# ZhangXinWhut/SimWhisper-Codec

Hardware: AMD Instinct MI355X
Metric: audio-sec/sec encode+decode (RTF^-1), 16kHz batch=32x10s (higher is better)
Workload: dtype split-f16 x3 encode (f32-class, f32 accumulate) / bf16 decode (f32 accumulate); 1 GPU; batch=32x10s @16kHz per GPU (32 utterances in all), encode()+decode(), 0.1*N(0,1) seed 1234, synthetic closed-form checkpoint (291M params); precision=mixed

## Files before the change

simwhisper_codec_amd/csrc/swc_gemm.hip:

```cpp
#include "swc_common.h"

static inline int tuning_env(const char* name, int dflt = 0) {
#ifdef SWC_TUNING
    const char* e = getenv(name);
    return e ? atoi(e) : dflt;
#else
    (void)name;
    return dflt;
#endif
}

namespace {


__device__ __attribute__((aligned(16))) unsigned int g_zero16[4] = {0u, 0u, 0u, 0u};
#ifdef SWC_GEMM_STAMP
__device__ unsigned long long g_stamps[512 * 8 * 8];
#endif

__device__ __forceinline__ void glds16(const void* gsrc, unsigned lds_addr) {
    unsigned keep;
    lds_addr = __builtin_amdgcn_readfirstlane(lds_addr);
    asm volatile(
        "s_mov_b32 %0, m0\n\ts_mov_b32 m0, %2\n\ts_nop 0\n\tglobal_load_lds_dwordx4 %1, off\n\ts_mov_b32 m0, %0"
        : "=&s"(keep)
        : "v"(gsrc), "s"(lds_addr)
        : "memory");
}
__device__ __forceinline__ void glds16_s(const char* base, unsigned off, unsigned lds_addr) {
    unsigned keep;
    lds_addr = __builtin_amdgcn_readfirstlane(lds_addr);
    asm volatile(
        "s_mov_b32 %0, m0\n\ts_mov_b32 m0, %3\n\ts_nop 0\n\tglobal_load_lds_dwordx4 %1, %2\n\ts_mov_b32 m0, %0"
        : "=&s"(keep)
        : "v"(off), "s"(base), "s"(lds_addr)
        : "memory");
}
__device__ __forceinline__ unsigned lds_addr_of(const void* p) {
    return (unsigned)(uintptr_t)(const __attribute__((address_space(3))) char*)p;
}

__device__ __forceinline__ int swz(int row) { return ((row >> 1) ^ ((row >> 4) << 1)) & 7; }
__device__ __forceinline__ int swz64(int row) { return ((-(row >> 2)) ^ (-(row >> 4))) & 3; }
template <int RB>
__device__ __forceinline__ int swz_rb(int row) { return RB == 128 ? swz(row) : swz64(row); }
template <int RB>
__device__ __forceinline__ int lds_off(int row, int chunk) { return row * RB + ((chunk ^ swz_rb<RB>(row)) << 4); }


struct GemmP {
    const char* A;
    const char* W;
    void* C;
    const float* bias;
    const float* gamma;
    const float* residual;
    long lda, ldw, ldc, ldr;
    int M, N, K;
    int taps, dil, stride, pad, t_in, t_out;
    int act;
    float alpha, out_scale;
    int band;
    unsigned* sat;
    int kc_per_tap;
    int n_tiles_n, n_tiles_m;
    int nt_mode;
    int stagger;
};

constexpr int EPI_TP = 68;
constexpr int EPI_WAVE_BYTES = 16 * EPI_TP * 4;


typedef unsigned u32x4_t __attribute__((ext_vector_type(4)));
typedef unsigned u32x2_t __attribute__((ext_vector_type(2)));
__device__ __forceinline__ void epi_st128(void* p, unsigned a, unsigned b, unsigned c, unsigned d, bool nt = false) {
#if defined(SWC_ABL_NOSTORE)
    asm volatile("" ::"v"(p), "v"(a), "v"(b), "v"(c), "v"(d));
#elif defined(SWC_EPI_PLAIN)
    (void)nt;
    *reinterpret_cast<uint4*>(p) = make_uint4(a, b, c, d);
#else
    if (nt) __builtin_nontemporal_store((u32x4_t){a, b, c, d}, reinterpret_cast<u32x4_t*>(p));
    else *reinterpret_cast<uint4*>(p) = make_uint4(a, b, c, d);
#endif
}
__device__ __forceinline__ void epi_st128f(void* p, float a, float b, float c, float d, bool nt = false) {
    epi_st128(p, __float_as_uint(a), __float_as_uint(b), __float_as_uint(c), __float_as_uint(d), nt);
}
__device__ __forceinline__ void epi_st64(void* p, unsigned a, unsigned b, bool nt = false) {
#if defined(SWC_ABL_NOSTORE)
    asm volatile("" ::"v"(p), "v"(a), "v"(b));
#elif defined(SWC_EPI_PLAIN)
    (void)nt;
    *reinterpret_cast<uint2*>(p) = make_uint2(a, b);
#else
    if (nt) __builtin_nontemporal_store((u32x2_t){a, b}, reinterpret_cast<u32x2_t*>(p));
    else *reinterpret_cast<uint2*>(p) = make_uint2(a, b);
#endif
}
__device__ __forceinline__ void epi_st32(void* p, unsigned a, bool nt = false) {
#if defined(SWC_ABL_NOSTORE)
    asm volatile("" ::"v"(p), "v"(a));
#elif defined(SWC_EPI_PLAIN)
    (void)nt;
    *reinterpret_cast<unsigned*>(p) = a;
#else
    if (nt) __builtin_nontemporal_store(a, reinterpret_cast<unsigned*>(p));
    else *reinterpret_cast<unsigned*>(p) = a;
#endif
}

template <typename OutT>
__device__ __forceinline__ float epi_act(float x) {
    return (__is_same(OutT, bf16_t) || __is_same(OutT, fp8_t)) ? gelu_fast(x) : (__is_same(OutT, f16s_t) ? gelu_as(x) : gelu_erf(x));
}

template <typename OutT, int MT, bool GELU>
__device__ __forceinline__ void gemm_epilogue_slab(const GemmP& p, f32x4 (&acc)[MT][4], int row0, int colw, int fr, int fh,
                                                   float* tbuf, float& amax, bool nt) {
    int lane = fr + 16 * fh;
    asm volatile("" : "+v"(lane));
    const int tr = lane >> 4, tc = (lane & 15) * 4;
    const int col = colw + tc;
    float4 b4 = make_float4(0.f, 0.f, 0.f, 0.f), g4 = make_float4(1.f, 1.f, 1.f, 1.f);
    if (p.bias) b4 = *reinterpret_cast<const float4*>(p.bias + col);
    if (p.gamma) g4 = *reinterpret_cast<const float4*>(p.gamma + col);
    float* wr_p = tbuf + (lane & 15) * EPI_TP + (lane >> 4) * 16;
    const float* rd_p = tbuf + tr * EPI_TP + tc;
#ifndef SWC_EPI_RD
#define SWC_EPI_RD 2
#endif
    constexpr int RD = SWC_EPI_RD < MT ? SWC_EPI_RD : MT - 1;
    float4 r4[MT][4];
    auto load_res = [&](int i) {
#pragma unroll
        for (int k = 0; k < 4; ++k) {
            const int row = row0 + 16 * i + tr + 4 * k;
            r4[i][k] = row < p.M ? *reinterpret_cast<const float4*>(p.residual + (long)row * p.ldr + col) : make_float4(0.f, 0.f, 0.f, 0.f);
        }
    };
    if (p.residual) {
#pragma unroll
        for (int i = 0; i < RD; ++i) load_res(i);
    }
#pragma unroll
    for (int i = 0; i < MT; ++i) {
        const int rbase = row0 + 16 * i + tr;
        if (p.residual && i + RD < MT) load_res(i + RD);
#pragma unroll
        for (int j = 0; j < 4; ++j) *reinterpret_cast<f32x4*>(wr_p + 4 * j) = acc[i][j];
        f32x4 t[4];
#pragma unroll
        for (int k = 0; k < 4; ++k) t[k] = *reinterpret_cast<const f32x4*>(rd_p + 4 * k * EPI_TP);
#pragma unroll
        for (int k = 0; k < 4; ++k) {
            const int row = rbase + 4 * k;
            float v0 = t[k][0] * p.alpha + b4.x, v1 = t[k][1] * p.alpha + b4.y, v2 = t[k][2] * p.alpha + b4.z, v3 = t[k][3] * p.alpha + b4.w;
            if constexpr (GELU) { v0 = epi_act<OutT>(v0); v1 = epi_act<OutT>(v1); v2 = epi_act<OutT>(v2); v3 = epi_act<OutT>(v3); }
            v0 *= g4.x; v1 *= g4.y; v2 *= g4.z; v3 *= g4.w;
            if (p.residual) { v0 += r4[i][k].x; v1 += r4[i][k].y; v2 += r4[i][k].z; v3 += r4[i][k].w; }
            if (row >= p.M) continue;
            if constexpr (__is_same(OutT, f16s_t)) {
                const float os = p.out_scale;
                f16s_store4(reinterpret_cast<unsigned short*>(p.C) + (long)row * p.ldc * 2, col, v0 * os, v1 * os, v2 * os, v3 * os, amax);
            } else if constexpr (sizeof(OutT) == 4) {
                epi_st128f(reinterpret_cast<float*>(p.C) + (long)row * p.ldc + col, v0, v1, v2, v3, nt);
            } else if constexpr (sizeof(OutT) == 1) {
                const float os = p.out_scale;
                epi_st32(reinterpret_cast<unsigned char*>(p.C) + (long)row * p.ldc + col, fp8_pack4(v0 * os, v1 * os, v2 * os, v3 * os, amax), nt);
            } else {
                epi_st64(reinterpret_cast<bf16_t*>(p.C) + (long)row * p.ldc + col, bf16_pack2(v0, v1), bf16_pack2(v2, v3), nt);
            }
        }
    }
}

template <typename OutT, int MT, int GELU>
__device__ __forceinline__ void gemm_epilogue_direct(const GemmP& p, f32x4 (&acc)[MT][4], int bm, int bn, int wr, int wc, int fr,
                                                     int fh, bool nt) {
    OutT* C = reinterpret_cast<OutT*>(p.C);
    const int col0 = bn + wc * 64 + 16 * fh;
    const bool vec_ok = (col0 + 16 <= p.N) && ((p.ldc & (sizeof(OutT) == 1 ? 15 : 3)) == 0) &&
                        (!p.residual || (p.ldr & 3) == 0) &&
                        ((reinterpret_cast<uintptr_t>(p.C) & 15) == 0) &&
                        ((reinterpret_cast<uintptr_t>(p.residual) & 15) == 0);
#ifdef SWC_KEEP_GAMMA16
    constexpr bool HAS_GAMMA = true;
#else
    constexpr bool HAS_GAMMA = sizeof(OutT) == 4;
#endif
    float bv[16], gv[HAS_GAMMA ? 16 : 1];
    float amax = 0.f;
    (void)amax; (void)gv;
    if (col0 + 16 <= p.N && ((reinterpret_cast<uintptr_t>(p.bias) | reinterpret_cast<uintptr_t>(p.gamma)) & 15) == 0) {
#pragma unroll
        for (int q = 0; q < 4; ++q) {
            const float4 b4 = p.bias ? *reinterpret_cast<const float4*>(p.bias + col0 + 4 * q) : make_float4(0.f, 0.f, 0.f, 0.f);
            bv[4 * q] = b4.x; bv[4 * q + 1] = b4.y; bv[4 * q + 2] = b4.z; bv[4 * q + 3] = b4.w;
            if constexpr (HAS_GAMMA) {
                const float4 g4 = p.gamma ? *reinterpret_cast<const float4*>(p.gamma + col0 + 4 * q) : make_float4(1.f, 1.f, 1.f, 1.f);
                gv[4 * q] = g4.x; gv[4 * q + 1] = g4.y; gv[4 * q + 2] = g4.z; gv[4 * q + 3] = g4.w;
            }
        }
    } else {
#pragma unroll
        for (int c = 0; c < 16; ++c) {
            const int col = col0 + c;
            bv[c] = (p.bias && col < p.N) ? p.bias[col] : 0.f;
            if constexpr (HAS_GAMMA) gv[c] = (p.gamma && col < p.N) ? p.gamma[col] : 1.f;
        }
    }
#pragma unroll
    for (int i = 0; i < MT; ++i) {
        const int row = bm + wr * (MT * 16) + i * 16 + fr;
        if (row >= p.M) continue;
        float v[16];
#pragma unroll
        for (int j = 0; j < 4; ++j)
#pragma unroll
            for (int e = 0; e < 4; ++e) v[4 * j + e] = acc[i][j][e] * p.alpha + bv[4 * j + e];
        if constexpr (GELU == 1) {
#pragma unroll
            for (int c = 0; c < 16; ++c) v[c] = epi_act<OutT>(v[c]);
        } else if constexpr (GELU == 2) {
#pragma unroll
            for (int c = 0; c < 16; ++c)
                if (p.act == SWC_ACT_GELU) v[c] = epi_act<OutT>(v[c]);
        }
        if constexpr (HAS_GAMMA) {
#pragma unroll
            for (int c = 0; c < 16; ++c) v[c] *= gv[c];
        }
        if constexpr (sizeof(OutT) == sizeof(f16s_t) && !__is_same(OutT, bf16_t)) {
            if (col0 + 16 <= p.N) {
                if (p.residual) {
                    const float4* rp = reinterpret_cast<const float4*>(p.residual + (long)row * p.ldr + col0);
#pragma unroll
                    for (int j = 0; j < 4; ++j) {
                        const float4 r4 = rp[j];
                        v[4 * j] += r4.x; v[4 * j + 1] += r4.y; v[4 * j + 2] += r4.z; v[4 * j + 3] += r4.w;
                    }
                }
                unsigned short* rowp = reinterpret_cast<unsigned short*>(p.C) + (long)row * p.ldc * 2;
                unsigned h2[8], l2[8];
#pragma unroll
                for (int c = 0; c < 8; ++c) f16s_split2(v[2 * c] * p.out_scale, v[2 * c + 1] * p.out_scale, h2[c], l2[c], amax);
                unsigned short* hp = rowp + f16s_col(col0);
#pragma unroll
                for (int q = 0; q < 2; ++q) {
                    epi_st128(reinterpret_cast<uint4*>(hp) + q, h2[4 * q], h2[4 * q + 1], h2[4 * q + 2], h2[4 * q + 3], nt);
                    epi_st128(reinterpret_cast<uint4*>(hp + 32) + q, l2[4 * q], l2[4 * q + 1], l2[4 * q + 2], l2[4 * q + 3], nt);
                }
            }
        } else if (vec_ok) {
            if (p.residual) {
                const float4* rp = reinterpret_cast<const float4*>(p.residual + (long)row * p.ldr + col0);
#pragma unroll
                for (int j = 0; j < 4; ++j) {
                    const float4 r4 = rp[j];
                    v[4 * j] += r4.x; v[4 * j + 1] += r4.y; v[4 * j + 2] += r4.z; v[4 * j + 3] += r4.w;
                }
            }
            OutT* cp = C + (long)row * p.ldc + col0;
            if constexpr (sizeof(OutT) == 4) {
#pragma unroll
                for (int j = 0; j < 4; ++j)
                    epi_st128f(reinterpret_cast<float4*>(cp) + j, v[4 * j], v[4 * j + 1], v[4 * j + 2], v[4 * j + 3], nt);
            } else if constexpr (sizeof(OutT) == 1) {
                const float os = p.out_scale;
                const unsigned u0 = fp8_pack4(v[0] * os, v[1] * os, v[2] * os, v[3] * os, amax);
                const unsigned u1 = fp8_pack4(v[4] * os, v[5] * os, v[6] * os, v[7] * os, amax);
                const unsigned u2 = fp8_pack4(v[8] * os, v[9] * os, v[10] * os, v[11] * os, amax);
                const unsigned u3 = fp8_pack4(v[12] * os, v[13] * os, v[14] * os, v[15] * os, amax);
                epi_st128(cp, u0, u1, u2, u3, nt);
            } else {
#pragma unroll
                for (int j = 0; j < 2; ++j)
                    epi_st128(reinterpret_cast<uint4*>(cp) + j, bf16_pack2(v[8 * j + 0], v[8 * j + 1]), bf16_pack2(v[8 * j + 2], v[8 * j + 3]),
                              bf16_pack2(v[8 * j + 4], v[8 * j + 5]), bf16_pack2(v[8 * j + 6], v[8 * j + 7]), nt);
            }
        } else {
#pragma unroll
            for (int c = 0; c < 16; ++c) {
                const int col = col0 + c;
                if (col >= p.N) continue;
                float x = v[c];
                if (p.residual) x += p.residual[(long)row * p.ldr + col];
                if constexpr (__is_same(OutT, fp8_t)) { x *= p.out_scale; amax = fmaxf(amax, fabsf(x)); }
                if constexpr (!__is_same(OutT, f16s_t)) store_out<OutT>(C + (long)row * p.ldc + col, x);
            }
        }
    }
    if constexpr (__is_same(OutT, f16s_t)) sat_commit(p.sat, 0, amax, SWC_F16S_LIMIT);
    if constexpr (__is_same(OutT, fp8_t)) sat_commit(p.sat, 1, amax, SWC_FP8_LIMIT);
}

template <typename OutT, int MT, bool SLAB, int ACT>
__device__ __forceinline__ void gemm_epilogue(const GemmP& p, f32x4 (&acc)[MT][4], int bm, int bn, int wr, int wc, int fr,
                                              int fh, float* tbuf, bool nt) {
    const bool gelu = ACT == 1 || (ACT == 2 && p.act == SWC_ACT_GELU);
    if constexpr (SLAB && sizeof(OutT) == 4 && !__is_same(OutT, f16s_t)) {
        const int colw = bn + wc * 64;
        const bool al16 = ((reinterpret_cast<uintptr_t>(p.C) | reinterpret_cast<uintptr_t>(p.residual) |
                            reinterpret_cast<uintptr_t>(p.bias) | reinterpret_cast<uintptr_t>(p.gamma)) & 15) == 0;
        const bool ok = tbuf && colw + 64 <= p.N && al16 && (p.ldc & (sizeof(OutT) == 1 ? 15 : 3)) == 0 &&
                        (!p.residual || (p.ldr & 3) == 0);
        if (__builtin_amdgcn_readfirstlane((int)ok)) {
            float amax = 0.f;
            if (gelu) gemm_epilogue_slab<OutT, MT, true>(p, acc, bm + wr * (MT * 16), colw, fr, fh, tbuf, amax, nt);
            else gemm_epilogue_slab<OutT, MT, false>(p, acc, bm + wr * (MT * 16), colw, fr, fh, tbuf, amax, nt);
            if constexpr (__is_same(OutT, fp8_t)) sat_commit(p.sat, 1, amax, SWC_FP8_LIMIT);
            return;
        }
    }
    if constexpr (ACT != 2) {
        gemm_epilogue_direct<OutT, MT, ACT>(p, acc, bm, bn, wr, wc, fr, fh, nt);
    } else if constexpr (__is_same(OutT, f16s_t) && MT == 8) {
        gemm_epilogue_direct<OutT, MT, 2>(p, acc, bm, bn, wr, wc, fr, fh, nt);
    } else {
        if (gelu) gemm_epilogue_direct<OutT, MT, 1>(p, acc, bm, bn, wr, wc, fr, fh, nt);
        else gemm_epilogue_direct<OutT, MT, 0>(p, acc, bm, bn, wr, wc, fr, fh, nt);
    }
}

template <int MODE, typename OutT, int MT, int WAVES_M, int WAVES_N, bool PLAIN, int RB = 128, int ACT = 2>
__global__ __launch_bounds__(WAVES_M* WAVES_N * 64, 2) void gemm_kernel(GemmP p) {
    constexpr int ROW_BYTES = RB;
    constexpr int CPR = RB / 16;
    constexpr int NG = RB / 64;
    static_assert(RB == 128 || (RB == 64 && MODE != SWC_F16S), "split-f16 needs hi|lo in one 128-byte row");
    static_assert(WAVES_M * WAVES_N * EPI_WAVE_BYTES <= (WAVES_M * MT * 16 + WAVES_N * 64) * RB, "epilogue scratch must fit one stage");
    constexpr bool BF16 = MODE == SWC_BF16;
    constexpr bool F16S = MODE == SWC_F16S;
    constexpr bool FP8 = MODE == SWC_FP8;
    constexpr int ES = BF16 ? 2 : (FP8 ? 1 : 4);
    constexpr int EPC = 16 / ES;
    constexpr int BK = ROW_BYTES / ES;
    constexpr int NT = WAVES_M * WAVES_N * 64;
    constexpr int BM = WAVES_M * MT * 16;
    constexpr int BN = WAVES_N * 64;
    constexpr int RPS = NT / CPR;
    constexpr int NA = BM / RPS;
    constexpr int NB = BN / RPS;
    constexpr int A_BYTES = BM * ROW_BYTES;
    constexpr int STAGE_BYTES = (BM + BN) * ROW_BYTES;

    extern __shared__ __attribute__((aligned(16))) char smem[];

    const int tid = threadIdx.x;
    const int lane = tid & 63;
    const int wave = tid >> 6;
    const int wr = wave / WAVES_N, wc = wave % WAVES_N;

    const int ntiles = p.n_tiles_m * p.n_tiles_n;
    const int xcd = blockIdx.x & 7;
    const int gw = ((int)gridDim.x - xcd + 7) >> 3;
    const int cq = ntiles >> 3, cr = ntiles & 7;
    const int chunk_start = xcd < cr ? xcd * (cq + 1) : cr * (cq + 1) + (xcd - cr) * cq;
    const int chunk_size = cq + (xcd < cr ? 1 : 0);
    int tl = blockIdx.x >> 3;
    if (tl >= chunk_size) return;
    int bm, bn;
    auto tile_origin = [&](int local) {
        const int bid = chunk_start + local;
        const int BAND = p.band;
        const int band = bid / (BAND * p.n_tiles_n);
        const int rem = bid - band * (BAND * p.n_tiles_n);
        const int rows_in_band = (p.n_tiles_m - band * BAND) < BAND ? (p.n_tiles_m - band * BAND) : BAND;
        const int tn = rem / rows_in_band;
        const int tm = band * BAND + (rem - tn * rows_in_band);
        bm = tm * BM;
        bn = tn * BN;
    };

    const int ld_pos = tid % CPR;
    const int ld_row = tid / CPR;
    int a_b[NA], a_t[NA], a_chunk[NA];
    bool a_rowok[NA];
    long w_rowoff[NB];
    int w_chunk[NB];
    bool w_rowok[NB];
    const int wave_u = __builtin_amdgcn_readfirstlane(wave);
    const unsigned smem_base = __builtin_amdgcn_readfirstlane(lds_addr_of(smem));
    constexpr int NV = RPS >= 64 ? 1 : 64 / RPS;
    unsigned chunkoff[NV];
#pragma unroll
    for (int v = 0; v < NV; ++v) chunkoff[v] = (unsigned)(ld_pos ^ swz_rb<RB>(ld_row + RPS * v)) << 4;
    const unsigned lda_bytes = (unsigned)(p.lda * ES), ldw_bytes = (unsigned)(p.ldw * ES);
    const char* a_base = p.A;
    const char* w_base = p.W;
    int a_left = 1, w_left = 1;
    auto setup_tile = [&](int local) {
        tile_origin(local);
        if constexpr (PLAIN) {
            a_base = p.A + (long)bm * lda_bytes;
            w_base = p.W + (long)bn * ldw_bytes;
            a_left = p.M - bm;
            w_left = p.N - bn;
            return;
        }
#pragma unroll
        for (int i = 0; i < NA; ++i) {
            const int row = ld_row + RPS * i;
            const int r = bm + row;
            const int chunk = ld_pos ^ swz_rb<RB>(row);
            if constexpr (!PLAIN) {
                a_rowok[i] = r < p.M;
                const int rr = a_rowok[i] ? r : 0;
                a_b[i] = rr / p.t_out;
                a_t[i] = rr - a_b[i] * p.t_out;
                a_chunk[i] = chunk;
            }
        }
#pragma unroll
        for (int i = 0; i < NB; ++i) {
            const int row = ld_row + RPS * i;
            const int n = bn + row;
            const int chunk = ld_pos ^ swz_rb<RB>(row);
            if constexpr (!PLAIN) {
                w_rowok[i] = n < p.N;
                w_rowoff[i] = (long)(w_rowok[i] ? n : 0) * p.ldw;
                w_chunk[i] = chunk;
            }
        }
    };
    setup_tile(tl);
    if (p.stagger > 0) {
        const int phase = (blockIdx.x >> 3) & 7;
        if (phase) {
            const unsigned long long t0 = __builtin_amdgcn_s_memtime();
            const unsigned long long wait = (unsigned long long)phase * (unsigned)p.stagger;
            while (__builtin_amdgcn_s_memtime() - t0 < wait) __builtin_amdgcn_s_sleep(32);
        }
    }
    auto stage_slice = [&](int kt, int stage) {
        const unsigned sa = smem_base + stage * STAGE_BYTES + wave_u * 1024;
        const unsigned sb = sa + A_BYTES;
        if constexpr (PLAIN) {
            const long koff = (long)kt * ROW_BYTES;
            const char* ab = a_base + koff;
            const char* wb = w_base + koff;
#pragma unroll
            for (int i = 0; i < NA; ++i) {
                const int r = min(ld_row + RPS * i, a_left - 1);
                glds16_s(ab, __umul24(r, lda_bytes) + chunkoff[i % NV], sa + RPS * i * ROW_BYTES);
            }
#pragma unroll
            for (int i = 0; i < NB; ++i) {
                const int r = min(ld_row + RPS * i, w_left - 1);
                glds16_s(wb, __umul24(r, ldw_bytes) + chunkoff[i % NV], sb + RPS * i * ROW_BYTES);
            }
            return;
        }
        const int tap = kt / p.kc_per_tap;
        const int kc = kt - tap * p.kc_per_tap;
        const int shift = tap * p.dil - p.pad;
        const char* zero = reinterpret_cast<const char*>(g_zero16);
#pragma unroll
        for (int i = 0; i < NA; ++i) {
            const int k0 = kc * BK + a_chunk[i] * EPC;
            const int ts = a_t[i] * p.stride + shift;
            const bool ok = a_rowok[i] && k0 < p.K && ts >= 0 && ts < p.t_in;
            const char* src = p.A + (((long)a_b[i] * p.t_in + (ok ? ts : 0)) * p.lda + (ok ? k0 : 0)) * ES;
            glds16(ok ? src : zero, sa + RPS * i * ROW_BYTES);
        }
#pragma unroll
        for (int i = 0; i < NB; ++i) {
            const int k0 = kc * BK + w_chunk[i] * EPC;
            const bool ok = w_rowok[i] && k0 < p.K;
            const char* src = p.W + (w_rowoff[i] + (long)tap * p.K + (ok ? k0 : 0)) * ES;
            glds16(ok ? src : zero, sb + RPS * i * ROW_BYTES);
        }
    };
#ifdef SWC_GEMM_STAMP
    unsigned long long st_last = 0, st_cmp = 0, st_vm = 0, st_bar = 0, st_n = 0;
    auto stamp = [&]() -> unsigned long long {
        unsigned long long t;
        asm volatile("s_memtime %0\n\ts_waitcnt lgkmcnt(0)" : "=s"(t)::"memory");
        return t;
    };
    auto dma_fence = [&]() {
        asm volatile("s_waitcnt lgkmcnt(0)" ::: "memory");
        const unsigned long long t1 = stamp();
        asm volatile("s_waitcnt vmcnt(0)" ::: "memory");
        const unsigned long long t2 = stamp();
        __syncthreads();
        const unsigned long long t3 = stamp();
        if (st_last) { st_cmp += t1 - st_last; st_vm += t2 - t1; st_bar += t3 - t2; st_n += 1; }
        st_last = t3;
    };
#else
    auto dma_fence = [&]() {
        asm volatile("s_waitcnt vmcnt(0)" ::: "memory");
        __syncthreads();
    };
#endif

    f32x4 acc[MT][4];
#pragma unroll
    for (int i = 0; i < MT; ++i)
#pragma unroll
        for (int j = 0; j < 4; ++j) acc[i][j] = (f32x4){0.f, 0.f, 0.f, 0.f};

    const int nkt = p.taps * p.kc_per_tap;
    const int fr = lane & 15, fh = lane >> 4;
    const int a_row0 = wr * (MT * 16) + fr;
    const int b_row0 = wc * 64 + 16 * (fr >> 2) + (fr & 3);
    stage_slice(0, 0);
    dma_fence();
#ifdef SWC_GEMM_PRIO47
    if (wave_u >= (WAVES_M * WAVES_N) / 2) __builtin_amdgcn_s_setprio(1);
#endif
    for (;;) {
    for (int kt = 0; kt < nkt; ++kt) {
        const int cur = kt & 1;
        if (kt + 1 < nkt) stage_slice(kt + 1, cur ^ 1);
#ifdef SWC_GEMM_IGLP
        __builtin_amdgcn_iglp_opt(SWC_GEMM_IGLP);
#endif
        const char* sa = smem + cur * STAGE_BYTES;
        const char* sb = sa + A_BYTES;
#ifdef SWC_GEMM_SPLIT
        constexpr bool EXPLICIT_SPLIT = (BF16 || F16S) && WAVES_M * WAVES_N == 8 && MT >= 4;
        constexpr int SPLIT = SWC_GEMM_SPLIT;
#else
        constexpr bool EXPLICIT_SPLIT = (F16S && WAVES_M * WAVES_N == 8 && MT >= 4) || ((BF16 || F16S) && WAVES_M * WAVES_N == 4);
        constexpr int SPLIT = WAVES_M * WAVES_N == 4 ? 0 : (MT == 8 ? 3 : 1);
#endif
        if constexpr (EXPLICIT_SPLIT) {
            uint4 f0a[MT], f0b[4], f1a[MT], f1b[4];
#pragma unroll
            for (int j = 0; j < 4; ++j) f0b[j] = *reinterpret_cast<const uint4*>(sb + lds_off<RB>(b_row0 + 4 * j, fh));
#pragma unroll
            for (int i = 0; i < MT; ++i) f0a[i] = *reinterpret_cast<const uint4*>(sa + lds_off<RB>(a_row0 + 16 * i, fh));
#pragma unroll
            for (int j = 0; j < 4; ++j) f1b[j] = *reinterpret_cast<const uint4*>(sb + lds_off<RB>(b_row0 + 4 * j, fh + 4));
#pragma unroll
            for (int i = 0; i < MT; ++i) f1a[i] = *reinterpret_cast<const uint4*>(sa + lds_off<RB>(a_row0 + 16 * i, fh + 4));
            auto mm = [&](int i) {
#pragma unroll
                for (int j = 0; j < 4; ++j) {
                    f32x4 c = acc[i][j];
                    if constexpr (F16S) {
                        c = __builtin_amdgcn_mfma_f32_16x16x32_f16(*reinterpret_cast<f16x8*>(&f1b[j]), *reinterpret_cast<f16x8*>(&f0a[i]), c, 0, 0, 0);
                        c = __builtin_amdgcn_mfma_f32_16x16x32_f16(*reinterpret_cast<f16x8*>(&f0b[j]), *reinterpret_cast<f16x8*>(&f1a[i]), c, 0, 0, 0);
                        c = __builtin_amdgcn_mfma_f32_16x16x32_f16(*reinterpret_cast<f16x8*>(&f0b[j]), *reinterpret_cast<f16x8*>(&f0a[i]), c, 0, 0, 0);
                    } else {
                        c = __builtin_amdgcn_mfma_f32_16x16x32_bf16(*reinterpret_cast<bf16x8*>(&f0b[j]), *reinterpret_cast<bf16x8*>(&f0a[i]), c, 0, 0, 0);
                        c = __builtin_amdgcn_mfma_f32_16x16x32_bf16(*reinterpret_cast<bf16x8*>(&f1b[j]), *reinterpret_cast<bf16x8*>(&f1a[i]), c, 0, 0, 0);
                    }
                    acc[i][j] = c;
                }
            };
#pragma unroll
            for (int i = 0; i < MT - SPLIT; ++i) mm(i);
            __builtin_amdgcn_sched_barrier(0);
            dma_fence();
            __builtin_amdgcn_sched_barrier(0);
#pragma unroll
            for (int i = MT - SPLIT; i < MT; ++i) mm(i);
            continue;
        }
        uint4 ha[(F16S || FP8) ? MT : 1], hb[(F16S || FP8) ? 4 : 1];
        (void)ha; (void)hb;
#pragma unroll
        for (int g = 0; g < NG; ++g) {
            uint4 fa[MT], fb[4];
#pragma unroll
            for (int j = 0; j < 4; ++j)
                fb[j] = *reinterpret_cast<const uint4*>(sb + lds_off<RB>(b_row0 + 4 * j, fh + 4 * g));
#pragma unroll
            for (int i = 0; i < MT; ++i)
                fa[i] = *reinterpret_cast<const uint4*>(sa + lds_off<RB>(a_row0 + 16 * i, fh + 4 * g));
            if constexpr (F16S) {
                if (g == 0) {
#pragma unroll
                    for (int i = 0; i < MT; ++i) ha[i] = fa[i];
#pragma unroll
                    for (int j = 0; j < 4; ++j) hb[j] = fb[j];
                } else {
#pragma unroll
                    for (int i = 0; i < MT; ++i)
#pragma unroll
                        for (int j = 0; j < 4; ++j) {
                            f32x4 c = acc[i][j];
                            c = __builtin_amdgcn_mfma_f32_16x16x32_f16(*reinterpret_cast<f16x8*>(&fb[j]),
                                                                       *reinterpret_cast<f16x8*>(&ha[i]), c, 0, 0, 0);
                            c = __builtin_amdgcn_mfma_f32_16x16x32_f16(*reinterpret_cast<f16x8*>(&hb[j]),
                                                                       *reinterpret_cast<f16x8*>(&fa[i]), c, 0, 0, 0);
                            c = __builtin_amdgcn_mfma_f32_16x16x32_f16(*reinterpret_cast<f16x8*>(&hb[j]),
                                                                       *reinterpret_cast<f16x8*>(&ha[i]), c, 0, 0, 0);
                            acc[i][j] = c;
                        }
                }
            } else if constexpr (BF16) {
#pragma unroll
                for (int i = 0; i < MT; ++i)
#pragma unroll
                    for (int j = 0; j < 4; ++j)
                        acc[i][j] = __builtin_amdgcn_mfma_f32_16x16x32_bf16(
                            *reinterpret_cast<bf16x8*>(&fb[j]), *reinterpret_cast<bf16x8*>(&fa[i]), acc[i][j], 0, 0, 0);
            } else if constexpr (FP8) {
                if (g == 0) {
#pragma unroll
                    for (int i = 0; i < MT; ++i) ha[i] = fa[i];
#pragma unroll
                    for (int j = 0; j < 4; ++j) hb[j] = fb[j];
                } else {
#pragma unroll
                    for (int i = 0; i < MT; ++i)
#pragma unroll
                        for (int j = 0; j < 4; ++j) {
                            i32x8 wa, xa;
                            wa[0] = hb[j].x; wa[1] = hb[j].y; wa[2] = hb[j].z; wa[3] = hb[j].w;
                            wa[4] = fb[j].x; wa[5] = fb[j].y; wa[6] = fb[j].z; wa[7] = fb[j].w;
                            xa[0] = ha[i].x; xa[1] = ha[i].y; xa[2] = ha[i].z; xa[3] = ha[i].w;
                            xa[4] = fa[i].x; xa[5] = fa[i].y; xa[6] = fa[i].z; xa[7] = fa[i].w;
                            acc[i][j] = __builtin_amdgcn_mfma_scale_f32_16x16x128_f8f6f4(wa, xa, acc[i][j], 0, 0, 0, 0x7f7f7f7f, 0,
                                                                                         0x7f7f7f7f);
                        }
                }
            } else {
#pragma unroll
                for (int e = 0; e < 4; ++e)
#pragma unroll
                    for (int i = 0; i < MT; ++i) {
                        const float av = __uint_as_float(reinterpret_cast<const unsigned*>(&fa[i])[e]);
#pragma unroll
                        for (int j = 0; j < 4; ++j) {
                            const float bv = __uint_as_float(reinterpret_cast<const unsigned*>(&fb[j])[e]);
                            acc[i][j] = __builtin_amdgcn_mfma_f32_16x16x4f32(bv, av, acc[i][j], 0, 0, 0);
                        }
                    }
            }
        }
        dma_fence();
    }
    const int bm_done = bm, bn_done = bn;
    tl += gw;
    const bool more = tl < chunk_size;
    if (more) {
        setup_tile(tl);
        stage_slice(0, 0);
    }
#ifdef SWC_GEMM_STAMP
    const unsigned long long st_e0 = stamp();
#endif
    gemm_epilogue<OutT, MT, MT < 8, ACT>(p, acc, bm_done, bn_done, wr, wc, fr, fh,
                            reinterpret_cast<float*>(smem + STAGE_BYTES + wave_u * EPI_WAVE_BYTES),
                            p.nt_mode == 2 || (p.nt_mode == 1 && !more));
#ifdef SWC_GEMM_STAMP
    asm volatile("s_waitcnt vmcnt(0)" ::: "memory");
    const unsigned long long st_e1 = stamp();
    if (lane == 0 && blockIdx.x < 512) {
        unsigned long long* o = g_stamps + ((long)blockIdx.x * 8 + wave) * 8;
        o[0] += st_cmp; o[1] += st_vm; o[2] += st_bar; o[3] += st_n; o[4] += st_e1 - st_e0; o[5] += 1; o[6] += st_e0 - st_last;
    }
    st_cmp = st_vm = st_bar = st_n = 0; st_last = 0;
#endif
    if (!more) break;
#pragma unroll
    for (int i = 0; i < MT; ++i)
#pragma unroll
        for (int j = 0; j < 4; ++j) acc[i][j] = (f32x4){0.f, 0.f, 0.f, 0.f};
    dma_fence();
    }
}

template <int MODE, typename OutT, int MT, int WM, int WN, bool PLAIN, int RB = 128, int ACT = 2>
int launch_k(GemmP p, hipStream_t s) {
    constexpr int BM = WM * MT * 16, BN = WN * 64;
    constexpr int LDS = 2 * (BM + BN) * RB;
    {
        constexpr int BK = RB / (MODE == SWC_BF16 ? 2 : (MODE == SWC_FP8 ? 1 : 4));
        p.kc_per_tap = (p.K + BK - 1) / BK;
    }
    p.n_tiles_n = (p.N + BN - 1) / BN;
    p.n_tiles_m = (p.M + BM - 1) / BM;
    {
        const int forced = tuning_env("SWC_GEMM_BAND");
        p.band = forced > 0 ? forced : (p.n_tiles_n >= 12 ? 4 : 1);
    }
    const long nwg = (long)p.n_tiles_n * p.n_tiles_m;
    if (nwg >= (1L << 30)) {
        swc_set_error("swc_gemm: grid too large");
        return SWC_E_ARG;
    }
    auto kern = gemm_kernel<MODE, OutT, MT, WM, WN, PLAIN, RB, ACT>;
    if (LDS > 64 * 1024) SWC_ENABLE_LDS(kern, LDS, "swc_gemm");
    const int persist = tuning_env("SWC_GEMM_NOPERSIST") ? 0 : 1;
    const long slots = 256L * (WM * WN == 4 ? 2 : 1);
    const long grid = (persist && nwg > slots) ? slots : nwg;
    p.nt_mode = tuning_env("SWC_GEMM_NT", 0);
    hipLaunchKernelGGL(kern, dim3((unsigned)grid), dim3(WM * WN * 64), LDS, s, p);
    return SWC_OK;
}

template <int MODE, typename OutT, int MT, int WM, int WN, int RB = 128>
int launch(GemmP p, hipStream_t s) {
    constexpr int BK = RB / (MODE == SWC_BF16 ? 2 : (MODE == SWC_FP8 ? 1 : 4));
    const long es = MODE == SWC_BF16 ? 2 : (MODE == SWC_FP8 ? 1 : 4);
    const bool plain = (p.taps == 1) && (p.K % BK == 0) && (p.stride == 1) && (p.pad == 0) && (p.t_in == p.t_out) &&
                       p.lda * es < (1L << 24) && p.ldw * es < (1L << 24);
    if constexpr (sizeof(OutT) < 4 && MODE != SWC_F32) {
        if (plain) return p.act == SWC_ACT_GELU ? launch_k<MODE, OutT, MT, WM, WN, true, RB, 1>(p, s) : launch_k<MODE, OutT, MT, WM, WN, true, RB, 0>(p, s);
        return launch_k<MODE, OutT, MT, WM, WN, false, RB, 2>(p, s);
    } else {
        return plain ? launch_k<MODE, OutT, MT, WM, WN, true, RB>(p, s) : launch_k<MODE, OutT, MT, WM, WN, false, RB>(p, s);
    }
}

}

static int tile_override() { return tuning_env("SWC_GEMM_TILE"); }

extern "C" int swc_gemm(const swc_gemm_args* a, void* stream) {
    SWC_CHECK_ARG(a != nullptr, "swc_gemm: null args");
    SWC_CHECK_ARG(a->A && a->W && a->C, "swc_gemm: null operand");
    SWC_CHECK_ARG(a->M >= 0 && a->N > 0 && a->K > 0, "swc_gemm: bad M/N/K %d %d %d", a->M, a->N, a->K);
    SWC_CHECK_ARG(a->a_dtype == SWC_F32 || a->a_dtype == SWC_BF16 || a->a_dtype == SWC_F16S || a->a_dtype == SWC_FP8,
                  "swc_gemm: bad a_dtype");
    SWC_CHECK_ARG(a->c_dtype == SWC_F32 || a->c_dtype == SWC_BF16 || a->c_dtype == SWC_F16S ||
                      (a->c_dtype == SWC_FP8 && a->a_dtype == SWC_FP8),
                  "swc_gemm: bad c_dtype (FP8 outputs come from FP8 operands only)");
    SWC_CHECK_ARG(a->c_dtype != SWC_F16S || a->a_dtype != SWC_FP8, "swc_gemm: fp8 operands have no split-f16 output");
    SWC_CHECK_ARG(a->c_dtype != SWC_F16S || a->a_dtype != SWC_BF16, "swc_gemm: bf16 operands have no split-f16 output");
    SWC_CHECK_ARG(a->c_dtype != SWC_BF16 || a->a_dtype != SWC_F16S, "swc_gemm: split-f16 operands have no bf16 output");
    SWC_CHECK_ARG(a->c_dtype != SWC_F16S || (a->N % 32 == 0 && a->ldc % 32 == 0 && aligned16(a->C)),
                  "swc_gemm: split-f16 output needs N, ldc multiples of 32 (N=%d)", a->N);
    SWC_CHECK_ARG(a->act == SWC_ACT_NONE || a->act == SWC_ACT_GELU, "swc_gemm: bad act");
    SWC_CHECK_ARG(!a->gamma || a->c_dtype == SWC_F32, "swc_gemm: gamma (per-column output scale) exists for f32 outputs only");
    const bool bf = a->a_dtype == SWC_BF16;
    const bool fs = a->a_dtype == SWC_F16S;
    const bool f8 = a->a_dtype == SWC_FP8;
    const int epc = bf ? 8 : (fs ? 32 : (f8 ? 16 : 4));
    SWC_CHECK_ARG(a->K % epc == 0, "swc_gemm: K=%d not a multiple of %d", a->K, epc);
    SWC_CHECK_ARG(a->lda % epc == 0 && a->ldw % epc == 0, "swc_gemm: lda/ldw break 16-byte rows");
    SWC_CHECK_ARG(aligned16(a->A) && aligned16(a->W), "swc_gemm: A/W not 16-byte aligned");
    SWC_CHECK_ARG(a->taps >= 1 && a->stride >= 1 && a->dil >= 1 && a->t_in >= 1 && a->t_out >= 1,
                  "swc_gemm: bad conv geometry");
    SWC_CHECK_ARG(a->M % a->t_out == 0, "swc_gemm: M=%d not a multiple of t_out=%d", a->M, a->t_out);
    SWC_CHECK_ARG(a->ldw >= (int64_t)a->taps * a->K, "swc_gemm: ldw < taps*K");
    SWC_CHECK_ARG(a->lda >= a->K && a->ldc >= a->N, "swc_gemm: lda < K or ldc < N");
    SWC_CHECK_ARG(!a->residual || a->ldr >= a->N, "swc_gemm: ldr < N");
    if (a->M == 0) return SWC_OK;

    GemmP p;
    p.A = (const char*)a->A;
    p.W = (const char*)a->W;
    p.C = a->C;
    p.bias = a->bias;
    p.gamma = a->gamma;
    p.residual = a->residual;
    p.lda = a->lda; p.ldw = a->ldw; p.ldc = a->ldc; p.ldr = a->ldr;
    p.M = a->M; p.N = a->N; p.K = a->K;
    p.taps = a->taps; p.dil = a->dil; p.stride = a->stride; p.pad = a->pad;
    p.t_in = a->t_in; p.t_out = a->t_out;
    p.act = a->act;
    p.alpha = a->alpha == 0.0f ? 1.0f : a->alpha;
    p.out_scale = a->out_scale == 0.0f ? 1.0f : a->out_scale;
    const int bk = bf ? 64 : (f8 ? 128 : 32);
    p.kc_per_tap = (a->K + bk - 1) / bk;
    p.n_tiles_n = p.n_tiles_m = 0;
    p.nt_mode = -1;
    p.stagger = tuning_env("SWC_GEMM_STAGGER", 0);
    p.sat = swc_sat_counter();
    hipStream_t s = (hipStream_t)stream;
    const long big_tiles = (long)((a->M + 255) / 256) * ((a->N + 255) / 256);
    bool big = (bf || f8) && a->N >= 256 && big_tiles >= 96;
    if (tile_override() == 128) big = false;
    if (tile_override() == 256) big = bf || f8;
    int rc;
    const int cd = a->c_dtype;
#define SWC_LAUNCH(MODE, MT, WM, WN)                                                        \
    (cd == SWC_BF16 ? launch<MODE, bf16_t, MT, WM, WN>(p, s)                                 \
                    : (cd == SWC_F16S ? launch<MODE, f16s_t, MT, WM, WN>(p, s) : launch<MODE, float, MT, WM, WN>(p, s)))
#define SWC_LAUNCH_B(MT, WM, WN) (cd == SWC_BF16 ? launch<SWC_BF16, bf16_t, MT, WM, WN>(p, s) : launch<SWC_BF16, float, MT, WM, WN>(p, s))
#define SWC_LAUNCH_S(MT, WM, WN) (cd == SWC_F16S ? launch<SWC_F16S, f16s_t, MT, WM, WN>(p, s) : launch<SWC_F16S, float, MT, WM, WN>(p, s))
    int mt = 8;
    if (((bf || f8) && big) || (fs && a->N >= 256 && big_tiles >= 96)) {
        const int forced = tuning_env("SWC_GEMM_MT");
        const long ntn = (a->N + 255) / 256;
        double best = 1e30;
        for (int cand : {8, 6, 4}) {
            const long tiles = ((a->M + cand * 32 - 1) / (cand * 32)) * ntn;
            const double cost = (double)((tiles + 255) / 256) * (cand + 1.5);
            if (cost < best - 1e-9) { best = cost; mt = cand; }
        }
        if (forced == 8 || forced == 6 || forced == 4) mt = forced;
    }
    const int small_env = tuning_env("SWC_GEMM_SMALL", 1);
    const long tiles128 = (long)((a->M + 127) / 128) * ((a->N + 127) / 128);
    const bool half_rows = small_env && tiles128 < 384 && a->M >= 512;
    if (f8) {
#define SWC_LAUNCH8(MT, WM, WN)                                                   \
    (cd == SWC_BF16 ? launch<SWC_FP8, bf16_t, MT, WM, WN>(p, s)                     \
                    : (cd == SWC_FP8 ? launch<SWC_FP8, fp8_t, MT, WM, WN>(p, s) : launch<SWC_FP8, float, MT, WM, WN>(p, s)))
        if (big)
            rc = mt == 8 ? SWC_LAUNCH8(8, 2, 4) : (mt == 6 ? SWC_LAUNCH8(6, 2, 4) : SWC_LAUNCH8(4, 2, 4));
        else
            rc = SWC_LAUNCH8(4, 2, 2);
#undef SWC_LAUNCH8
    } else if (bf) {
        if (big)
            rc = mt == 8 ? SWC_LAUNCH_B(8, 2, 4) : (mt == 6 ? SWC_LAUNCH_B(6, 2, 4) : SWC_LAUNCH_B(4, 2, 4));
        else
            rc = half_rows ? SWC_LAUNCH_B(2, 2, 2) : SWC_LAUNCH_B(4, 2, 2);
    } else if (fs) {
        bool bigs = a->N >= 256 && big_tiles >= 96;
        if (tile_override() == 128) bigs = false;
        if (tile_override() == 256) bigs = true;
        if (bigs)
            rc = mt == 8 ? SWC_LAUNCH_S(8, 2, 4) : (mt == 6 ? SWC_LAUNCH_S(6, 2, 4) : SWC_LAUNCH_S(4, 2, 4));
        else
            rc = half_rows ? SWC_LAUNCH_S(2, 2, 2) : SWC_LAUNCH_S(4, 2, 2);
    } else {
        rc = SWC_LAUNCH(SWC_F32, 4, 2, 2);
    }
#undef SWC_LAUNCH
#undef SWC_LAUNCH_B
#undef SWC_LAUNCH_S
    if (rc != SWC_OK) return rc;
    SWC_CHECK_LAUNCH("swc_gemm");
    return SWC_OK;
}

#ifdef SWC_GEMM_STAMP
extern "C" int swc_debug_stamps(void* host_out, int reset) {
    if (host_out && hipMemcpyFromSymbol(host_out, HIP_SYMBOL(g_stamps), sizeof(unsigned long long) * 512 * 8 * 8) != hipSuccess) return -1;
    if (reset) {
        static unsigned long long zeros[512 * 8 * 8];
        if (hipMemcpyToSymbol(HIP_SYMBOL(g_stamps), zeros, sizeof(zeros)) != hipSuccess) return -1;
    }
    return 0;
}
#endif
```

Measured before the change: 15520 audio-s/s.

## Add intra-workgroup K-split GEMM variant for narrow bf16 multi-tap convolutions

Adds a KG template parameter so a workgroup runs KG groups of waves, each handling every KG-th K slice with its own LDS sub-stage. Partial accumulators are reduced through LDS before group 0 runs the epilogue. Selects KG=2 with small 2x2x2 tiles for bf16 multi-tap convs with f32 output, N<=512 and K span 3072-3584, to raise parallelism on small-N shapes. Costs are an extra LDS reduction with two barriers and one workgroup per CU.

```diff
diff --git a/simwhisper_codec_amd/csrc/swc_gemm.hip b/simwhisper_codec_amd/csrc/swc_gemm.hip
--- a/simwhisper_codec_amd/csrc/swc_gemm.hip
+++ b/simwhisper_codec_amd/csrc/swc_gemm.hip
@@ -324,13 +324,20 @@
     }
 }
 
-template <int MODE, typename OutT, int MT, int WAVES_M, int WAVES_N, bool PLAIN, int RB = 128, int ACT = 2>
-__global__ __launch_bounds__(WAVES_M* WAVES_N * 64, 2) void gemm_kernel(GemmP p) {
+template <int MODE, int MT, int WAVES_M, int WAVES_N, int RB, int KG>
+constexpr int gemm_lds_bytes() { return 2 * KG * (WAVES_M * MT * 16 + WAVES_N * 64) * RB; }
+constexpr int gemm_wg_per_cu(int waves, int kg) { return kg == 1 && waves == 4 ? 2 : 1; }
+
+template <int MODE, typename OutT, int MT, int WAVES_M, int WAVES_N, bool PLAIN, int RB = 128, int ACT = 2, int KG = 1>
+__global__ __launch_bounds__(KG* WAVES_M* WAVES_N * 64, (KG == 1 ? 2 : 1))
+void gemm_kernel(GemmP p) {
     constexpr int ROW_BYTES = RB;
     constexpr int CPR = RB / 16;
     constexpr int NG = RB / 64;
     static_assert(RB == 128 || (RB == 64 && MODE != SWC_F16S), "split-f16 needs hi|lo in one 128-byte row");
-    static_assert(WAVES_M * WAVES_N * EPI_WAVE_BYTES <= (WAVES_M * MT * 16 + WAVES_N * 64) * RB, "epilogue scratch must fit one stage");
+    static_assert(WAVES_M * WAVES_N * EPI_WAVE_BYTES <= KG * (WAVES_M * MT * 16 + WAVES_N * 64) * RB, "epilogue scratch must fit one stage");
+    static_assert(KG == 1 || (KG - 1) * WAVES_M * WAVES_N * MT * 4 * 1024 <= gemm_lds_bytes<MODE, MT, WAVES_M, WAVES_N, RB, KG>(),
+                  "the K-split partial tiles must fit the LDS");
     constexpr bool BF16 = MODE == SWC_BF16;
     constexpr bool F16S = MODE == SWC_F16S;
     constexpr bool FP8 = MODE == SWC_FP8;
@@ -344,11 +351,13 @@
     constexpr int NA = BM / RPS;
     constexpr int NB = BN / RPS;
     constexpr int A_BYTES = BM * ROW_BYTES;
-    constexpr int STAGE_BYTES = (BM + BN) * ROW_BYTES;
+    constexpr int SUB_BYTES = (BM + BN) * ROW_BYTES;
+    constexpr int STAGE_BYTES = KG * SUB_BYTES;
 
     extern __shared__ __attribute__((aligned(16))) char smem[];
 
-    const int tid = threadIdx.x;
+    const int kg = KG > 1 ? (int)__builtin_amdgcn_readfirstlane(threadIdx.x / NT) : 0;
+    const int tid = KG > 1 ? (int)threadIdx.x - kg * NT : (int)threadIdx.x;
     const int lane = tid & 63;
     const int wave = tid >> 6;
     const int wr = wave / WAVES_N, wc = wave % WAVES_N;
@@ -435,7 +444,7 @@
         }
     }
     auto stage_slice = [&](int kt, int stage) {
-        const unsigned sa = smem_base + stage * STAGE_BYTES + wave_u * 1024;
+        const unsigned sa = smem_base + stage * STAGE_BYTES + kg * SUB_BYTES + wave_u * 1024;
         const unsigned sb = sa + A_BYTES;
         if constexpr (PLAIN) {
             const long koff = (long)kt * ROW_BYTES;
@@ -503,29 +512,29 @@
 #pragma unroll
         for (int j = 0; j < 4; ++j) acc[i][j] = (f32x4){0.f, 0.f, 0.f, 0.f};
 
-    const int nkt = p.taps * p.kc_per_tap;
+    const int nks = p.taps * p.kc_per_tap / KG;
     const int fr = lane & 15, fh = lane >> 4;
     const int a_row0 = wr * (MT * 16) + fr;
     const int b_row0 = wc * 64 + 16 * (fr >> 2) + (fr & 3);
-    stage_slice(0, 0);
+    stage_slice(kg, 0);
     dma_fence();
 #ifdef SWC_GEMM_PRIO47
     if (wave_u >= (WAVES_M * WAVES_N) / 2) __builtin_amdgcn_s_setprio(1);
 #endif
     for (;;) {
-    for (int kt = 0; kt < nkt; ++kt) {
-        const int cur = kt & 1;
-        if (kt + 1 < nkt) stage_slice(kt + 1, cur ^ 1);
+    for (int ks = 0; ks < nks; ++ks) {
+        const int cur = ks & 1;
+        if (ks + 1 < nks) stage_slice((ks + 1) * KG + kg, cur ^ 1);
 #ifdef SWC_GEMM_IGLP
         __builtin_amdgcn_iglp_opt(SWC_GEMM_IGLP);
 #endif
-        const char* sa = smem + cur * STAGE_BYTES;
+        const char* sa = smem + cur * STAGE_BYTES + kg * SUB_BYTES;
         const char* sb = sa + A_BYTES;
 #ifdef SWC_GEMM_SPLIT
         constexpr bool EXPLICIT_SPLIT = (BF16 || F16S) && WAVES_M * WAVES_N == 8 && MT >= 4;
         constexpr int SPLIT = SWC_GEMM_SPLIT;
 #else
-        constexpr bool EXPLICIT_SPLIT = (F16S && WAVES_M * WAVES_N == 8 && MT >= 4) || ((BF16 || F16S) && WAVES_M * WAVES_N == 4);
+        constexpr bool EXPLICIT_SPLIT = (F16S && WAVES_M * WAVES_N == 8 && MT >= 4) || ((BF16 || F16S) && WAVES_M * WAVES_N == 4 && RB == 128);
         constexpr int SPLIT = WAVES_M * WAVES_N == 4 ? 0 : (MT == 8 ? 3 : 1);
 #endif
         if constexpr (EXPLICIT_SPLIT) {
@@ -637,19 +646,39 @@
         }
         dma_fence();
     }
+    if constexpr (KG > 1) {
+        f32x4* red = reinterpret_cast<f32x4*>(smem) + (wave * MT * 4) * 64 + lane;
+        constexpr int GROUP_SLOTS = WAVES_M * WAVES_N * MT * 4 * 64;
+        if (kg > 0) {
+#pragma unroll
+            for (int i = 0; i < MT; ++i)
+#pragma unroll
+                for (int j = 0; j < 4; ++j) red[(kg - 1) * GROUP_SLOTS + (i * 4 + j) * 64] = acc[i][j];
+        }
+        __syncthreads();
+        if (kg == 0) {
+            for (int g = 1; g < KG; ++g)
+#pragma unroll
+                for (int i = 0; i < MT; ++i)
+#pragma unroll
+                    for (int j = 0; j < 4; ++j) acc[i][j] += red[(g - 1) * GROUP_SLOTS + (i * 4 + j) * 64];
+        }
+        __syncthreads();
+    }
     const int bm_done = bm, bn_done = bn;
     tl += gw;
     const bool more = tl < chunk_size;
     if (more) {
         setup_tile(tl);
-        stage_slice(0, 0);
+        stage_slice(kg, 0);
     }
 #ifdef SWC_GEMM_STAMP
     const unsigned long long st_e0 = stamp();
 #endif
-    gemm_epilogue<OutT, MT, MT < 8, ACT>(p, acc, bm_done, bn_done, wr, wc, fr, fh,
-                            reinterpret_cast<float*>(smem + STAGE_BYTES + wave_u * EPI_WAVE_BYTES),
-                            p.nt_mode == 2 || (p.nt_mode == 1 && !more));
+    if (kg == 0)
+        gemm_epilogue<OutT, MT, MT < 8, ACT>(p, acc, bm_done, bn_done, wr, wc, fr, fh,
+                                reinterpret_cast<float*>(smem + STAGE_BYTES + wave_u * EPI_WAVE_BYTES),
+                                p.nt_mode == 2 || (p.nt_mode == 1 && !more));
 #ifdef SWC_GEMM_STAMP
     asm volatile("s_waitcnt vmcnt(0)" ::: "memory");
     const unsigned long long st_e1 = stamp();
@@ -668,10 +697,10 @@
     }
 }
 
-template <int MODE, typename OutT, int MT, int WM, int WN, bool PLAIN, int RB = 128, int ACT = 2>
+template <int MODE, typename OutT, int MT, int WM, int WN, bool PLAIN, int RB = 128, int ACT = 2, int KG = 1>
 int launch_k(GemmP p, hipStream_t s) {
     constexpr int BM = WM * MT * 16, BN = WN * 64;
-    constexpr int LDS = 2 * (BM + BN) * RB;
+    constexpr int LDS = gemm_lds_bytes<MODE, MT, WM, WN, RB, KG>();
     {
         constexpr int BK = RB / (MODE == SWC_BF16 ? 2 : (MODE == SWC_FP8 ? 1 : 4));
         p.kc_per_tap = (p.K + BK - 1) / BK;
@@ -687,27 +716,27 @@
         swc_set_error("swc_gemm: grid too large");
         return SWC_E_ARG;
     }
-    auto kern = gemm_kernel<MODE, OutT, MT, WM, WN, PLAIN, RB, ACT>;
+    auto kern = gemm_kernel<MODE, OutT, MT, WM, WN, PLAIN, RB, ACT, KG>;
     if (LDS > 64 * 1024) SWC_ENABLE_LDS(kern, LDS, "swc_gemm");
     const int persist = tuning_env("SWC_GEMM_NOPERSIST") ? 0 : 1;
-    const long slots = 256L * (WM * WN == 4 ? 2 : 1);
+    const long slots = 256L * gemm_wg_per_cu(WM * WN, KG);
     const long grid = (persist && nwg > slots) ? slots : nwg;
     p.nt_mode = tuning_env("SWC_GEMM_NT", 0);
-    hipLaunchKernelGGL(kern, dim3((unsigned)grid), dim3(WM * WN * 64), LDS, s, p);
+    hipLaunchKernelGGL(kern, dim3((unsigned)grid), dim3(KG * WM * WN * 64), LDS, s, p);
     return SWC_OK;
 }
 
-template <int MODE, typename OutT, int MT, int WM, int WN, int RB = 128>
+template <int MODE, typename OutT, int MT, int WM, int WN, int RB = 128, int KG = 1>
 int launch(GemmP p, hipStream_t s) {
     constexpr int BK = RB / (MODE == SWC_BF16 ? 2 : (MODE == SWC_FP8 ? 1 : 4));
     const long es = MODE == SWC_BF16 ? 2 : (MODE == SWC_FP8 ? 1 : 4);
     const bool plain = (p.taps == 1) && (p.K % BK == 0) && (p.stride == 1) && (p.pad == 0) && (p.t_in == p.t_out) &&
                        p.lda * es < (1L << 24) && p.ldw * es < (1L << 24);
     if constexpr (sizeof(OutT) < 4 && MODE != SWC_F32) {
-        if (plain) return p.act == SWC_ACT_GELU ? launch_k<MODE, OutT, MT, WM, WN, true, RB, 1>(p, s) : launch_k<MODE, OutT, MT, WM, WN, true, RB, 0>(p, s);
-        return launch_k<MODE, OutT, MT, WM, WN, false, RB, 2>(p, s);
+        if (plain) return p.act == SWC_ACT_GELU ? launch_k<MODE, OutT, MT, WM, WN, true, RB, 1, KG>(p, s) : launch_k<MODE, OutT, MT, WM, WN, true, RB, 0, KG>(p, s);
+        return launch_k<MODE, OutT, MT, WM, WN, false, RB, 2, KG>(p, s);
     } else {
-        return plain ? launch_k<MODE, OutT, MT, WM, WN, true, RB>(p, s) : launch_k<MODE, OutT, MT, WM, WN, false, RB>(p, s);
+        return plain ? launch_k<MODE, OutT, MT, WM, WN, true, RB, 2, KG>(p, s) : launch_k<MODE, OutT, MT, WM, WN, false, RB, 2, KG>(p, s);
     }
 }
 
@@ -793,7 +822,24 @@
     const int small_env = tuning_env("SWC_GEMM_SMALL", 1);
     const long tiles128 = (long)((a->M + 127) / 128) * ((a->N + 127) / 128);
     const bool half_rows = small_env && tiles128 < 384 && a->M >= 512;
-    if (f8) {
+    const long kspan = (long)a->taps * a->K;
+    const int kslices = a->taps * ((a->K + bk - 1) / bk);
+    const bool ks_shape = cd == SWC_F32 && a->N <= 512 && kspan >= 3072 && kspan <= 3584 && a->K % 64 == 0 && kslices % 4 == 0;
+    int ksplit = (bf && a->taps > 1 && ks_shape) ? 1 : 0;
+#ifdef SWC_TUNING
+    if (bf && ksplit) ksplit = tuning_env("SWC_GEMM_KSPLIT", 1);
+    if (fs && ks_shape) ksplit = tuning_env("SWC_GEMM_KSPLIT", 0);
+    if (ksplit && fs) {
+        rc = launch<SWC_F16S, float, 2, 2, 2, 128, 2>(p, s);
+    } else
+#endif
+    if (ksplit && bf) {
+#ifdef SWC_TUNING
+        if (ksplit == 2) rc = launch<SWC_BF16, float, 2, 2, 2, 64, 2>(p, s);
+        else
+#endif
+        rc = launch<SWC_BF16, float, 2, 2, 2, 128, 2>(p, s);
+    } else if (f8) {
 #define SWC_LAUNCH8(MT, WM, WN)                                                   \
     (cd == SWC_BF16 ? launch<SWC_FP8, bf16_t, MT, WM, WN>(p, s)                     \
                     : (cd == SWC_FP8 ? launch<SWC_FP8, fp8_t, MT, WM, WN>(p, s) : launch<SWC_FP8, float, MT, WM, WN>(p, s)))
```

New measurement: 15580 audio-s/s, median of 6. No clear change (+0.4%).
